# randyjhc/vit-colmap

Measured on AMD Instinct MI355X. Metric: images/sec extracted + pair-matches/sec (N×D brute-force NN), higher is better.
Workload: dtype bf16 (ViT) / u8+i32 (matcher); 1 GPU; configs[1]+configs[2]: DINOv2 ViT-S/14 extract of 50 640x480 images (512 keypoints, 384-D uint8 descriptors) then exhaustive mutual-NN + ratio matching of all pairs among the extracted images; images_total=50, images_rank0=50, num_keypoints=512, descriptor_dim=384, parallelism=images+pairs sharded x1

## Files before the change

vit_colmap_amd/csrc/gemm.hip:

```cpp
#include <hip/hip_runtime.h>
#include <stdint.h>

#include "../../include/vitcolmap_hip.h"
#include "common.h"
#include "device.h"

namespace {

typedef __bf16 v8bf __attribute__((ext_vector_type(8)));
typedef __bf16 v4bf __attribute__((ext_vector_type(4)));
typedef float v4f __attribute__((ext_vector_type(4)));

constexpr int BM = 128;
constexpr int BN = 128;
constexpr int BK = 64;
constexpr int kImg = 128 * 128;
constexpr int kStage = 2 * kImg;

enum { EPI_BIAS = 0, EPI_GELU = 1, EPI_RESIDUAL = 2, EPI_PATCH = 3, EPI_SWIGLU = 4 };
static_assert(EPI_BIAS == VC_EPI_BIAS && EPI_GELU == VC_EPI_GELU && EPI_RESIDUAL == VC_EPI_RESIDUAL && EPI_SWIGLU == VC_EPI_SWIGLU,
              "epilogue codes of the ABI");

__device__ __forceinline__ float gelu_erf(float x) {
  const float ax = __builtin_fabsf(x);
// ... 125 lines not shown
          *(v4bf*)(out + (size_t)m * H + n) = ov;
        }
      }
    }
    return;
  }
#pragma unroll
  for (int a = 0; a < 4; ++a) {
    const int n = n0 + wn * 64 + a * 16 + fq * 4;
    const v4bf bv = *(const v4bf*)(bias + n);
#pragma unroll
    for (int b = 0; b < 4; ++b) {
      const int m = m0 + wm * 64 + b * 16 + fr;
      if (m < M) {
        size_t o = (size_t)m * N + n;
        size_t ro = o;
        if (EPI == EPI_PATCH) {
          const int b_img = m / group;
          o = (size_t)(m + b_img + 1) * N + n;
          ro = (size_t)(m - b_img * group + 1) * N + n;
        }
        float v[4];
#pragma unroll
        for (int j = 0; j < 4; ++j) v[j] = acc[a][b][j] + (float)bv[j];
        if (EPI == EPI_GELU) {
#pragma unroll
          for (int j = 0; j < 4; ++j) v[j] = gelu_erf(v[j]);
        }
        if (EPI == EPI_RESIDUAL || EPI == EPI_PATCH) {
          const v4bf rv = *(const v4bf*)(res + ro);
#pragma unroll
          for (int j = 0; j < 4; ++j) v[j] += (float)rv[j];
        }
        v4bf ov;
#pragma unroll
        for (int j = 0; j < 4; ++j) ov[j] = (__bf16)v[j];
        *(v4bf*)(out + o) = ov;
      }
    }
  }
}


constexpr int G2M = 256, G2N = 256;
constexpr int kUnit2 = 128 * 128;
constexpr int kBuf2 = 4 * kUnit2;
constexpr int G256_LDS = 2 * kBuf2;
constexpr int kAhead2 = 6;

template <int EPI, bool CONV>
__global__ __launch_bounds__(512, 2) void gemm256_kernel(const __bf16* __restrict__ X, const __bf16* __restrict__ W,
                                                         const __bf16* __restrict__ bias, const __bf16* __restrict__ res,
                                                         __bf16* __restrict__ out, int M, int N, int K, int n_tiles_n,
                                                         int n_tiles, int cH, int cW, int cC, int ckw, int cdy0, int cdx0,
                                                         int cpar) {
  extern __shared__ __attribute__((aligned(1024))) uint8_t lds2[];
  const int tid = threadIdx.x, lane = tid & 63;
  const int wave = __builtin_amdgcn_readfirstlane(tid >> 6);
  const int wr = wave >> 2, wc = wave & 3;
  const int nk = K / BK;
  const int n_units = 4 * nk;
  for (int slot = blockIdx.x; slot < n_tiles; slot += gridDim.x) {
  int tile;
  {
    const int xcd = slot & 7, idx = slot >> 3;
    const int q = n_tiles >> 3, r = n_tiles & 7;
    tile = (xcd < r ? xcd * (q + 1) : r * (q + 1) + (xcd - r) * q) + idx;
  }
  const int tm = tile / n_tiles_n, tn = tile - tm * n_tiles_n;
  const int m0 = tm * G2M, n0 = tn * G2N;

  const uint32_t lds0 = vc::lds_addr(&lds2[0]);
  const int prow = lane >> 3, pchunk = (lane & 7) ^ prow;
  uint32_t voffx[2][2], voffw[2];
  uint32_t vtaps[2][2];
  const int n_taps = CONV ? K / cC : 1, tiles_per_tap = CONV ? cC / BK : 1;
#pragma unroll
  for (int i = 0; i < 2; ++i) {
    const int rho = (wave * 2 + i) * 8 + prow;
#pragma unroll
    for (int h = 0; h < 2; ++h) {
      const int xr = (rho < 64 ? rho : 128 + (rho - 64)) + 64 * h;
      if (CONV) {
        const int m = m0 + xr, hw = cH * cW;
        const int bimg = m / hw, rem = m - bimg * hw, py = rem / cW, px = rem - py * cW;
        uint32_t bits = 0;
        for (int t = 0; t < n_taps; ++t) {
          const int yy = py + cdy0 + t / ckw, xx = px + cdx0 + t % ckw;
          if (m < M && yy >= 0 && yy < cH && xx >= 0 && xx < cW) bits |= 1u << t;
        }
        vtaps[h][i] = bits;
        voffx[h][i] = (uint32_t)(((size_t)min(m, M - 1) * cC + pchunk * 8) * 2);
      } else {
        voffx[h][i] = (uint32_t)(((size_t)min(m0 + xr, M - 1) * K + pchunk * 8) * 2 - (size_t)min(m0, M - 1) * K * 2);
      }
    }
    const int wrow = EPI == EPI_SWIGLU ? rho : (rho >> 5) * 64 + (rho & 31);
    voffw[i] = (uint32_t)(((size_t)wrow * K + pchunk * 8) * 2);
  }
  const int H = N >> 1, j0 = tn * (G2N / 2);
  const char* const xbase = CONV ? (const char*)X : (const char*)(X + (size_t)min(m0, M - 1) * K);
  const char* const wbase = (const char*)(W + (size_t)(EPI == EPI_SWIGLU ? j0 : n0) * K);
  const size_t whalf = (size_t)(EPI == EPI_SWIGLU ? H : 32) * K * 2;
  auto issue = [&](int u) {
    if (u >= n_units) return;
    const int t = u >> 2, j = u & 3;
    const bool is_x = j == 0 || j == 3;
    const char* sb = is_x ? xbase + (size_t)t * (BK * 2) : wbase + (size_t)t * (BK * 2) + (j == 2 ? whalf : 0);
    int tap = 0;
    uint32_t zoff = 0, spos = 0;
    if (CONV && is_x) {
      tap = t / tiles_per_tap;
      const long long shift = ((long long)(cdy0 + tap / ckw) * cW + (cdx0 + tap % ckw)) * cC * 2;
      const long long sneg = shift < 0 ? shift : 0;
      spos = (uint32_t)(shift - sneg);
      sb = xbase + sneg + (long long)(t - tap * tiles_per_tap) * (BK * 2);
      zoff = (uint32_t)((long long)M * cC * 2 - sneg) + (uint32_t)pchunk * 16u;
    }
#pragma unroll
    for (int i = 0; i < 2; ++i) {
      uint32_t vo = j == 0 ? voffx[0][i] : (j == 3 ? voffx[1][i] : voffw[i]);
      if (CONV && is_x) vo = ((j == 0 ? vtaps[0][i] : vtaps[1][i]) >> tap) & 1u ? vo + spos : zoff;
      const uint32_t dst = lds0 + (uint32_t)(t & 1) * kBuf2 + (uint32_t)j * kUnit2 + (uint32_t)(wave * 2 + i) * 1024u;
      vc::lds_dma16(sb, vo, dst);
    }
  };

  v4f acc[4][8];
#pragma unroll
  for (int a = 0; a < 4; ++a)
#pragma unroll
    for (int b = 0; b < 8; ++b) acc[a][b] = (v4f){0.f, 0.f, 0.f, 0.f};

  const int fr = lane & 15, fq = lane >> 4;
  uint32_t xoff[2], woff[2];
#pragma unroll
  for (int ks = 0; ks < 2; ++ks) {
    const int ch = ks * 4 + fq;
    xoff[ks] = (uint32_t)(wr * 64 + fr) * 128u + (uint32_t)((ch ^ (fr & 7)) << 4);
    woff[ks] = (uint32_t)(wc * 32 + fr) * 128u + (uint32_t)((ch ^ (fr & 7)) << 4);
  }
  v8bf xf[2][4], wf[2][2][2];

  auto read_x = [&](const uint8_t* buf, int th) {
    const uint8_t* u = buf + (th == 0 ? 0 : 3) * kUnit2;
#pragma unroll
    for (int ks = 0; ks < 2; ++ks)
#pragma unroll
      for (int b = 0; b < 4; ++b) xf[ks][b] = *(const v8bf*)(u + xoff[ks] + b * 2048);
  };
  auto read_w = [&](const uint8_t* buf, int fh) {
    const uint8_t* u = buf + (1 + fh) * kUnit2;
#pragma unroll
    for (int ks = 0; ks < 2; ++ks)
#pragma unroll
      for (int a = 0; a < 2; ++a) wf[fh][ks][a] = *(const v8bf*)(u + woff[ks] + a * 2048);
  };
  auto barrier = []() { asm volatile("s_barrier" ::: "memory"); };
#define G2_MFMA(FH, TH)                                                                                      \
  asm volatile("s_waitcnt lgkmcnt(0)" ::: "memory");                                                         \
  __builtin_amdgcn_sched_barrier(0);                                                                         \
  __builtin_amdgcn_s_setprio(1);                                                                             \
  _Pragma("unroll") for (int ks = 0; ks < 2; ++ks)                                                           \
  _Pragma("unroll") for (int a = 0; a < 2; ++a)                                                              \
  _Pragma("unroll") for (int b = 0; b < 4; ++b)                                                              \
    acc[2 * (FH) + a][4 * (TH) + b] =                                                                        \
        __builtin_amdgcn_mfma_f32_16x16x32_bf16(wf[FH][ks][a], xf[ks][b], acc[2 * (FH) + a][4 * (TH) + b], 0, 0, 0); \
  __builtin_amdgcn_s_setprio(0);

#pragma unroll
  for (int u = 0; u < kAhead2; ++u) issue(u);
  if (nk > 1) asm volatile("s_waitcnt vmcnt(4)" ::: "memory"); else asm volatile("s_waitcnt vmcnt(0)" ::: "memory");
  barrier();
  if (wr == 1) barrier();

  for (int t = 0; t < nk; ++t) {
    const uint8_t* buf = lds2 + (size_t)(t & 1) * kBuf2;
    const int g = 4 * t;
    read_w(buf, 0);
    __builtin_amdgcn_sched_barrier(0);
    read_x(buf, 0);
    issue(g + kAhead2);
    barrier();
    G2_MFMA(0, 0)
    barrier();
    read_w(buf, 1);
    issue(g + 1 + kAhead2);
    barrier();
    G2_MFMA(1, 0)
    barrier();
    read_x(buf, 1);
    issue(g + 2 + kAhead2);
    barrier();
    G2_MFMA(1, 1)
    barrier();
    issue(g + 3 + kAhead2);
    if (t + 2 < nk) asm volatile("s_waitcnt vmcnt(4)" ::: "memory"); else asm volatile("s_waitcnt vmcnt(0)" ::: "memory");
    barrier();
    G2_MFMA(0, 1)
    barrier();
  }
  if (wr == 0) barrier();
#undef G2_MFMA

  typedef unsigned int v4u32 __attribute__((ext_vector_type(4)));
  typedef unsigned int v2u32 __attribute__((ext_vector_type(2)));
  typedef __bf16 v2bf16 __attribute__((ext_vector_type(2)));
  uint8_t* const ep = lds2 + (size_t)wave * 16384;
  const int lrow = lane >> 3, lslot = lane & 7;
  auto ep_at = [&](int row, int byte) { return ep + row * 128 + (byte ^ (((row >> 1) & 7) << 4)); };
  if (EPI == EPI_SWIGLU) {
    const size_t colh = (size_t)j0 + wc * 32;
#pragma unroll
    for (int a = 0; a < 2; ++a) {
      const v4bf bg = *(const v4bf*)(bias + colh + a * 16 + fq * 4), bv = *(const v4bf*)(bias + H + colh + a * 16 + fq * 4);
#pragma unroll
      for (int b = 0; b < 8; ++b) {
        const int row = 16 * b + fr;
        float v[4];
#pragma unroll
        for (int j = 0; j < 4; ++j) v[j] = swiglu_f32(acc[a][b][j] + (float)bg[j], acc[a + 2][b][j] + (float)bv[j]);
        const v2bf16 q0 = {(__bf16)v[0], (__bf16)v[1]}, q1 = {(__bf16)v[2], (__bf16)v[3]};
        *(v2u32*)ep_at(row >> 1, 64 * (row & 1) + 32 * a + 8 * fq) = (v2u32){*(const unsigned int*)&q0, *(const unsigned int*)&q1};
      }
    }
    asm volatile("s_waitcnt lgkmcnt(0)" ::: "memory");
#pragma unroll
    for (int i = 0; i < 8; ++i) {
      const int m = m0 + wr * 128 + 16 * i + (lane >> 2);
      const v4u32 o = *(const v4u32*)ep_at(8 * i + lrow, lslot * 16);
      if (m < M) *(v4u32*)(out + (size_t)m * H + colh + (lane & 3) * 8) = o;
    }
    asm volatile("s_barrier" ::: "memory");
    continue;
  }
  const size_t col0 = (size_t)n0 + wc * 64;
  if (EPI == EPI_RESIDUAL) {
    v4u32 rr[16];
#pragma unroll
    for (int i = 0; i < 16; ++i)
      rr[i] = *(const v4u32*)(res + (size_t)min(m0 + wr * 128 + 8 * i + lrow, M - 1) * N + col0 + lslot * 8);
#pragma unroll
    for (int i = 0; i < 16; ++i) *(v4u32*)ep_at(8 * i + lrow, lslot * 16) = rr[i];
    asm volatile("s_waitcnt lgkmcnt(0)" ::: "memory");
  }
#pragma unroll
  for (int a = 0; a < 4; ++a) {
    const v4bf bv = *(const v4bf*)(bias + col0 + a * 16 + fq * 4);
#pragma unroll
    for (int b = 0; b < 8; ++b) {
      uint8_t* const pp = ep_at(16 * b + fr, 32 * a + 8 * fq);
      float v[4];
#pragma unroll
      for (int j = 0; j < 4; ++j) v[j] = acc[a][b][j] + (float)bv[j];
      if (EPI == EPI_GELU) {
#pragma unroll
        for (int j = 0; j < 4; j += 2) {
          const v2f_t g = gelu_erf2((v2f_t){v[j], v[j + 1]});
          v[j] = g[0];
          v[j + 1] = g[1];
        }
      }
      if (EPI == EPI_RESIDUAL) {
        const v2u32 r8 = *(const v2u32*)pp;
#pragma unroll
        for (int j = 0; j < 2; ++j) {
          v[2 * j] += __uint_as_float(r8[j] << 16);
          v[2 * j + 1] += __uint_as_float(r8[j] & 0xffff0000u);
        }
      }
      const v2bf16 q0 = {(__bf16)v[0], (__bf16)v[1]}, q1 = {(__bf16)v[2], (__bf16)v[3]};
      *(v2u32*)pp = (v2u32){*(const unsigned int*)&q0, *(const unsigned int*)&q1};
    }
  }
  asm volatile("s_waitcnt lgkmcnt(0)" ::: "memory");
  if (CONV && cpar >= 0) {
    int mm = m0 + wr * 128 + lrow;
    int pb = mm / (cH * cW), py = (mm - pb * cH * cW) / cW, px = mm - pb * cH * cW - py * cW;
#pragma unroll
    for (int i = 0; i < 16; ++i) {
      const int row = 8 * i + lrow;
      const v4u32 o = *(const v4u32*)ep_at(row, lslot * 16);
      const size_t orow = ((size_t)pb * 2 * cH + 2 * py + (cpar >> 1)) * (2 * cW) + 2 * px + (cpar & 1);
      if (mm < M) *(v4u32*)(out + orow * N + col0 + lslot * 8) = o;
      mm += 8;
      px += 8;
      while (px >= cW) { px -= cW; if (++py == cH) { py = 0; ++pb; } }
    }
  } else {
#pragma unroll
    for (int i = 0; i < 16; ++i) {
      const int row = 8 * i + lrow, m = m0 + wr * 128 + row;
      const v4u32 o = *(const v4u32*)ep_at(row, lslot * 16);
      if (m < M) *(v4u32*)(out + (size_t)m * N + col0 + lslot * 8) = o;
    }
  }
  asm volatile("s_barrier" ::: "memory");
  }
}

constexpr int XK = 384;
constexpr int XKS = XK / 16;
constexpr int XStage = XKS * 1024;
constexpr int XNS = 3;
constexpr int XPF = XNS - 1;
constexpr int XMaxN = 4096;
constexpr int XRows = 256;
constexpr int XChunk = 32 * 128;
constexpr int XOffBias = XNS * XStage;
constexpr int XOffStage = XOffBias + XMaxN * 4;
constexpr int XLds = XOffStage + 8 * 2 * XChunk;

typedef float v16f __attribute__((ext_vector_type(16)));
typedef uint32_t v4u __attribute__((ext_vector_type(4)));

constexpr uint32_t kGtLo = (127 - 14) << 7;
constexpr uint32_t kGtN = 17 * 128;
constexpr int kGtBytes = (int)kGtN * 2 * 2;

__device__ __forceinline__ uint32_t f32_to_bf16_rne(float v) {
  uint32_t u = __float_as_uint(v);
  u += 0x7fffu + ((u >> 16) & 1u);
  return u >> 16;
}
__global__ void gelu_table_kernel(uint16_t* __restrict__ tab) {
  const uint32_t i = blockIdx.x * blockDim.x + threadIdx.x;
  if (i >= kGtN * 2) return;
  const uint32_t k = i >> 1, sign = i & 1;
  const float x = __uint_as_float(((sign << 15) | (kGtLo + k)) << 16);
  const float y = 0.5f * x * (1.0f + erff(x * 0.70710678118654752f));
  tab[i] = (uint16_t)f32_to_bf16_rne(y);
}

constexpr int XReadAhead = 8;
constexpr int XIssue0 = 1;
constexpr int XIssueStep = 8;
template <int EPI, bool LN, bool GT>
__global__ __launch_bounds__(512, 1) void xs_kernel(const __bf16* __restrict__ X, const uint8_t* __restrict__ Wp,
                                                    const float* __restrict__ biasf, const __bf16* res,
                                                    __bf16* out, int M, int N, int n_nb, int n_stages, float eps,
                                                    const uint16_t* __restrict__ gelu_tab) {
  __shared__ __attribute__((aligned(1024))) uint8_t lds[XLds];
  const int tid = threadIdx.x, lane = tid & 63;
  const int wave = __builtin_amdgcn_readfirstlane(tid >> 6);
  const int r = lane & 31, h = lane >> 5;

  const int G = gridDim.x, bid = blockIdx.x;
  const int s0 = (int)((long long)n_stages * bid / G), s1 = (int)((long long)n_stages * (bid + 1) / G);
  const int n = s1 - s0;
  if (n <= 0) return;

  float* bias_l = (float*)(lds + XOffBias);
  for (int i = tid; i < N; i += 512) bias_l[i] = biasf[i];
  uint8_t* const gt_l = lds + XOffBias + ((N * 4 + 15) & ~15);
  if (GT)
    for (int i = tid; i < kGtBytes / 4; i += 512) ((uint32_t*)gt_l)[i] = ((const uint32_t*)gelu_tab)[i];

  const uint32_t lds0 = vc::lds_addr(&lds[0]);
  int inb = s0 % n_nb, islot = 0, ileft = n;
  const uint32_t lane_off16 = (uint32_t)lane * 16u;
  auto issue_piece = [&](int i) {
    const uint8_t* sbase = Wp + (size_t)inb * XStage + (size_t)(wave * 3 + i) * 1024;
    const uint32_t dst = lds0 + (uint32_t)islot * XStage + (uint32_t)(wave * 3 + i) * 1024u;
    vc::lds_dma16(sbase, lane_off16, dst);
    if (i == 2) {
      if (ileft > 1) { --ileft; inb = inb + 1 == n_nb ? 0 : inb + 1; }
      islot = islot + 1 == XNS ? 0 : islot + 1;
    }
  };
  auto issue = [&]() {
#pragma unroll
    for (int i = 0; i < 3; ++i) issue_piece(i);
  };
#pragma unroll
  for (int j = 0; j < XPF; ++j) issue();

  v8bf xf[XKS];
  typedef float v2f __attribute__((ext_vector_type(2)));
  const int prow = lane >> 3;
  auto x_issue = [&](int mt) {
#pragma unroll
    for (int p = 0; p < 4; ++p) {
      const int m = min(mt * XRows + wave * 32 + 8 * p + prow, M - 1);
      const uint8_t* src = (const uint8_t*)X + (size_t)m * (XK * 2) + (lane & 7) * 16;
#pragma unroll
      for (int c = 0; c < XK / 64; ++c) *(v4u*)&xf[4 * c + p] = *(const v4u*)(src + c * 128);
    }
  };
  auto x_finish = [&]() {
    uint8_t* const tp = lds + XOffStage + wave * (2 * XChunk);
    const int fsw = (r >> 1) & 7;
#pragma unroll
    for (int c = 0; c < XK / 64; ++c) {
#pragma unroll
      for (int p = 0; p < 4; ++p) {
        const int row = 8 * p + prow;
        *(v4u*)(tp + row * 128 + (((lane & 7) ^ ((row >> 1) & 7)) << 4)) = *(const v4u*)&xf[4 * c + p];
      }
#pragma unroll
      for (int k4 = 0; k4 < 4; ++k4)
        xf[4 * c + k4] = *(const v8bf*)(tp + r * 128 + (((2 * k4 + h) ^ fsw) << 4));
    }
    if (LN) {
      auto expand = [](uint32_t u) { return (v2f){__uint_as_float(u << 16), __uint_as_float(u & 0xffff0000u)}; };
      v2f s2 = {0.f, 0.f};
#pragma unroll
      for (int ks = 0; ks < XKS; ++ks) {
        const v4u u = *(const v4u*)&xf[ks];
#pragma unroll
        for (int j = 0; j < 4; ++j) s2 += expand(u[j]);
      }
      float sum = s2[0] + s2[1];
      sum += __shfl_xor(sum, 32);
      const float mean = sum * (1.0f / XK);
      const v2f mean2 = {mean, mean};
#pragma unroll
      for (int ks = 0; ks < XKS; ++ks) asm volatile("" : "+v"(xf[ks]));
      v2f q2 = {0.f, 0.f};
#pragma unroll
      for (int ks = 0; ks < XKS; ++ks) {
        const v4u u = *(const v4u*)&xf[ks];
#pragma unroll
        for (int j = 0; j < 4; ++j) { const v2f d = expand(u[j]) - mean2; q2 = __builtin_elementwise_fma(d, d, q2); }
      }
      float q = q2[0] + q2[1];
      q += __shfl_xor(q, 32);
      const float rstd = __builtin_amdgcn_rsqf(q * (1.0f / XK) + eps);
      const v2f rstd2 = {rstd, rstd};
#pragma unroll
      for (int ks = 0; ks < XKS; ++ks) asm volatile("" : "+v"(xf[ks]));
#pragma unroll
      for (int ks = 0; ks < XKS; ++ks) {
        const v4u u = *(const v4u*)&xf[ks];
#pragma unroll
        for (int j = 0; j < 4; ++j) {
          const v2f y = (expand(u[j]) - mean2) * rstd2;
          xf[ks][2 * j] = (__bf16)y[0];
          xf[ks][2 * j + 1] = (__bf16)y[1];
        }
      }
    }
  };

  const __amdgpu_buffer_rsrc_t out_rs = __builtin_amdgcn_make_buffer_rsrc(out, 0, (int)((size_t)M * N * 2), 0x00020000);
  uint8_t* const tr_out = lds + XOffStage + wave * (2 * XChunk);
  uint8_t* const tr_res = tr_out + 2048;
  const int crow = lane >> 2, cch = lane & 3;
  const int rsw = (r >> 2) & 3;
  v4u resq[2];
  auto load_res = [&](int m_base, int nb) {
    if (EPI == EPI_RESIDUAL) {
#pragma unroll
      for (int q = 0; q < 2; ++q)
        resq[q] = *(const v4u*)(res + (size_t)min(m_base + crow + 16 * q, M - 1) * N + nb * 32 + cch * 8);
    }
  };
  v16f pa;
  float ev[16];
  uint32_t ep[8];
  v4u eo[2];
  int pm_base = 0, pnb = 0;
  auto res_to_lds = [&]() {
    if (EPI == EPI_RESIDUAL) {
#pragma unroll
      for (int q = 0; q < 2; ++q) {
        const int row = crow + 16 * q;
        *(v4u*)(tr_res + row * 64 + ((cch ^ ((row >> 2) & 3)) << 4)) = resq[q];
      }
    }
  };
  uint32_t gq[8];
  uint32_t gres[8];
  uint32_t gbad = 0;
  auto slice = [&](int sl) {
    if (EPI == EPI_GELU && GT) {
      typedef __bf16 v2bf __attribute__((ext_vector_type(2)));
      if (sl < 4) {
        const int g = sl;
        const v2bf lo = {(__bf16)pa[4 * g], (__bf16)pa[4 * g + 1]}, hi = {(__bf16)pa[4 * g + 2], (__bf16)pa[4 * g + 3]};
        ep[2 * g] = *(const uint32_t*)&lo;
        ep[2 * g + 1] = *(const uint32_t*)&hi;
        if (sl == 0) gbad = 0;
      }
      if (sl >= 4 && sl < 12) {
        const int qd = sl - 4;
        const uint32_t b0 = ep[qd] & 0xffffu, b1 = ep[qd] >> 16;
        const uint32_t k0 = (b0 & 0x7fffu) - kGtLo, k1 = (b1 & 0x7fffu) - kGtLo;
        gbad = max(gbad, max(k0, k1));
        const uint32_t a0 = min(k0, kGtN - 1) * 4 + ((b0 >> 15) << 1), a1 = min(k1, kGtN - 1) * 4 + ((b1 >> 15) << 1);
        gq[2 * (qd & 3)] = *(const uint16_t*)(gt_l + a0);
        gq[2 * (qd & 3) + 1] = *(const uint16_t*)(gt_l + a1);
      }
      if (sl >= 7 && sl < 15) {
        const int qd = sl - 7;
        gres[qd] = gq[2 * (qd & 3)] | (gq[2 * (qd & 3) + 1] << 16);
      }
      if (sl == 15) {
        if (__any(gbad >= kGtN)) {
#pragma unroll
          for (int qd = 0; qd < 8; ++qd) {
            const v2f_t xin = {__uint_as_float(ep[qd] << 16), __uint_as_float(ep[qd] & 0xffff0000u)};
            const v2f_t y = gelu_erf2(xin);
            const v2bf o = {(__bf16)y[0], (__bf16)y[1]};
            ep[qd] = *(const uint32_t*)&o;
          }
        } else {
#pragma unroll
          for (int qd = 0; qd < 8; ++qd) ep[qd] = gres[qd];
        }
      }
      if (sl == 16) {
#pragma unroll
        for (int i = 0; i < 4; ++i) {
          const auto sw = __builtin_amdgcn_permlane32_swap(ep[i], ep[i + 4], false, false);
          ep[i] = sw[0];
          ep[i + 4] = sw[1];
        }
      }
      if (sl == 17) {
        *(v4u*)(tr_out + r * 64 + (((2 * h) ^ rsw) << 4)) = (v4u){ep[0], ep[1], ep[4], ep[5]};
        *(v4u*)(tr_out + r * 64 + (((2 * h + 1) ^ rsw) << 4)) = (v4u){ep[2], ep[3], ep[6], ep[7]};
      }
      if (sl == 19) {
#pragma unroll
        for (int q = 0; q < 2; ++q) {
          const int row = crow + 16 * q;
          eo[q] = *(const v4u*)(tr_out + row * 64 + ((cch ^ ((row >> 2) & 3)) << 4));
        }
      }
      if (sl == 22) {
#pragma unroll
        for (int q = 0; q < 2; ++q) {
          const int row = crow + 16 * q;
          __builtin_amdgcn_raw_buffer_store_b128(eo[q], out_rs, (int)(((size_t)(pm_base + row) * N + pnb * 32 + cch * 8) * 2), 0, 0);
        }
      }
      return;
    }
    if (sl < 8) {
      const int j0 = 2 * sl;
      if (EPI == EPI_GELU) {
        const v2f_t y = gelu_erf2((v2f_t){pa[j0], pa[j0 + 1]});
        ev[j0] = y[0];
        ev[j0 + 1] = y[1];
      } else if (EPI == EPI_RESIDUAL) {
        if ((sl & 1) == 0) {
          const int g = sl >> 1;
          const v4bf rv = *(const v4bf*)(tr_res + r * 64 + ((g ^ rsw) << 4) + 8 * h);
#pragma unroll
          for (int j = 0; j < 4; ++j) ev[4 * g + j] = pa[4 * g + j] + (float)rv[j];
        }
      } else {
        ev[j0] = pa[j0];
        ev[j0 + 1] = pa[j0 + 1];
      }
    } else if (sl < 12) {
      const int g = sl - 8;
      typedef __bf16 v2bf __attribute__((ext_vector_type(2)));
      const v2bf lo = {(__bf16)ev[4 * g], (__bf16)ev[4 * g + 1]}, hi = {(__bf16)ev[4 * g + 2], (__bf16)ev[4 * g + 3]};
      ep[2 * g] = *(const uint32_t*)&lo;
      ep[2 * g + 1] = *(const uint32_t*)&hi;
    } else if (sl == 12) {
#pragma unroll
      for (int i = 0; i < 4; ++i) {
        const auto sw = __builtin_amdgcn_permlane32_swap(ep[i], ep[i + 4], false, false);
        ep[i] = sw[0];
        ep[i + 4] = sw[1];
      }
    } else if (sl == 13) {
      *(v4u*)(tr_out + r * 64 + (((2 * h) ^ rsw) << 4)) = (v4u){ep[0], ep[1], ep[4], ep[5]};
      *(v4u*)(tr_out + r * 64 + (((2 * h + 1) ^ rsw) << 4)) = (v4u){ep[2], ep[3], ep[6], ep[7]};
    } else if (sl == 15) {
#pragma unroll
      for (int q = 0; q < 2; ++q) {
        const int row = crow + 16 * q;
        eo[q] = *(const v4u*)(tr_out + row * 64 + ((cch ^ ((row >> 2) & 3)) << 4));
      }
    } else if (sl == 19) {
#pragma unroll
      for (int q = 0; q < 2; ++q) {
        const int row = crow + 16 * q;
        __builtin_amdgcn_raw_buffer_store_b128(eo[q], out_rs, (int)(((size_t)(pm_base + row) * N + pnb * 32 + cch * 8) * 2), 0, 0);
      }
    }
  };

  v16f acc;
  int mt_cur = -1, slot = 0;
  int mt = s0 / n_nb, nb = s0 - mt * n_nb;
  for (int i = 0; i < n; ++i) {
    if (i >= 2) {
      if (EPI == EPI_RESIDUAL) asm volatile("s_waitcnt vmcnt(7)" ::: "memory");
      else asm volatile("s_waitcnt vmcnt(5)" ::: "memory");
    } else {
      asm volatile("s_waitcnt vmcnt(3)" ::: "memory");
    }
    asm volatile("s_waitcnt lgkmcnt(0)\n\ts_barrier" ::: "memory");
    const bool pending = i > 0;
    if (pending) res_to_lds();
    const bool reload = mt != mt_cur;
    const int m_base = mt * XRows + wave * 32;
    if (reload) {
      x_issue(mt);
      if (pending) {
#pragma unroll
        for (int sl = 0; sl < XKS; ++sl) slice(sl);
      }
      x_finish();
      mt_cur = mt;
    }
    load_res(m_base, nb);
    const uint8_t* st = lds + slot * XStage + lane * 16;
    {
      const float* bl = bias_l + nb * 32 + 4 * h;
#pragma unroll
      for (int g = 0; g < 4; ++g) {
        const v4f bv = *(const v4f*)(bl + 8 * g);
#pragma unroll
        for (int j = 0; j < 4; ++j) acc[4 * g + j] = bv[j];
      }
    }
    {
      constexpr int XRD = (EPI == EPI_GELU && GT) ? 6 : XReadAhead;
      v8bf wf[XKS];
#pragma unroll
      for (int ks = 0; ks < XRD; ++ks) wf[ks] = *(const v8bf*)(st + ks * 1024);
      __builtin_amdgcn_sched_barrier(0);
      if (pending && !reload) {
#pragma unroll
        for (int ks = 0; ks < XKS; ++ks) {
          acc = __builtin_amdgcn_mfma_f32_32x32x16_bf16(wf[ks], xf[ks], acc, 0, 0, 0);
          if (ks + XRD < XKS) wf[ks + XRD] = *(const v8bf*)(st + (ks + XRD) * 1024);
          slice(ks);
          if (ks == XIssue0 || ks == XIssue0 + XIssueStep || ks == XIssue0 + 2 * XIssueStep)
            issue_piece((ks - XIssue0) / XIssueStep);
          __builtin_amdgcn_sched_barrier(0);
        }
      } else {
#pragma unroll
        for (int ks = 0; ks < XKS; ++ks) {
          acc = __builtin_amdgcn_mfma_f32_32x32x16_bf16(wf[ks], xf[ks], acc, 0, 0, 0);
          if (ks + XRD < XKS) wf[ks + XRD] = *(const v8bf*)(st + (ks + XRD) * 1024);
          if (ks == XIssue0 || ks == XIssue0 + XIssueStep || ks == XIssue0 + 2 * XIssueStep)
            issue_piece((ks - XIssue0) / XIssueStep);
          __builtin_amdgcn_sched_barrier(0);
        }
      }
    }
    pa = acc;
    pm_base = m_base;
    pnb = nb;
    slot = slot + 1 == XNS ? 0 : slot + 1;
    if (++nb == n_nb) { nb = 0; ++mt; }
  }
  res_to_lds();
#pragma unroll
  for (int sl = 0; sl < XKS; ++sl) slice(sl);
  asm volatile("s_waitcnt vmcnt(0)" ::: "memory");
}

__global__ __launch_bounds__(256) void xs_prepare_kernel(const float* __restrict__ W, const float* __restrict__ b,
                                                         const float* __restrict__ gamma, const float* __restrict__ beta,
                                                         int N, __bf16* __restrict__ Wp, float* __restrict__ biasf) {
  const int lane = threadIdx.x & 63;
  const int nfeat = blockIdx.x * 4 + (threadIdx.x >> 6);
  if (nfeat >= N) return;
  const int nb = nfeat >> 5, rr = nfeat & 31;
  float dot = 0.f;
  for (int k = lane; k < XK; k += 64) {
    const float w = W[(size_t)nfeat * XK + k];
    const float wg = gamma ? w * gamma[k] : w;
    if (beta) dot += w * beta[k];
    const int ks = k >> 4, hh = (k >> 3) & 1, j = k & 7;
    Wp[(((size_t)nb * XKS + ks) * 64 + hh * 32 + rr) * 8 + j] = (__bf16)wg;
  }
#pragma unroll
  for (int o = 32; o > 0; o >>= 1) dot += __shfl_xor(dot, o);
  if (lane == 0) biasf[nfeat] = (b ? b[nfeat] : 0.f) + dot;
}


constexpr int MStage = 2 * XStage;
constexpr int MNS = 2;

constexpr int M2OffB1 = MNS * MStage;
constexpr int M2OffGt = M2OffB1 + 1536 * 4;
constexpr int M2OffB2 = M2OffGt + 8704;
constexpr int M2OffTrA = M2OffB2 + 1536;
constexpr int M2OffTrB = M2OffTrA + 4 * XChunk;
constexpr int M2OffG = M2OffTrB + 4 * XChunk;
constexpr int M2Lds = M2OffG + 2 * 4 * 2048;
static_assert(M2Lds <= 160 * 1024, "fused MLP: LDS budget");

constexpr int M2ReadAhead = 6;
constexpr int M2PiecesA = 3;
constexpr int M2Issue0 = 1;
constexpr int M2IssueStep = 3;
constexpr int M2IssueStepB = 2;
__global__ __launch_bounds__(512, 2) void mlp2_kernel(__bf16* __restrict__ X, const uint8_t* __restrict__ Wm,
                                                      const float* __restrict__ b1f, const float* __restrict__ b2f,
                                                      int M, int n_chunks, int n_tiles, float eps,
                                                      const uint16_t* __restrict__ gelu_tab) {
  __shared__ __attribute__((aligned(1024))) uint8_t lds[M2Lds];
  const int tid = threadIdx.x, lane = tid & 63;
  const int wave = __builtin_amdgcn_readfirstlane(tid >> 6);
  const bool roleB = wave >= 4;
  const int pairw = wave & 3;
  const int r = lane & 31, h = lane >> 5;
  const int G = gridDim.x, bid = blockIdx.x;
  const int my_tiles = bid < n_tiles ? (n_tiles - bid + G - 1) / G : 0;
  const int n = my_tiles * n_chunks;
  if (n <= 0) return;

  float* const b1_l = (float*)(lds + M2OffB1);
  float* const b2_l = (float*)(lds + M2OffB2);
  uint8_t* const gt_l = lds + M2OffGt;
  for (int i = tid; i < n_chunks * 32; i += 512) b1_l[i] = b1f[i];
  for (int i = tid; i < XK; i += 512) b2_l[i] = b2f[i];
  for (int i = tid; i < kGtBytes / 4; i += 512) ((uint32_t*)gt_l)[i] = ((const uint32_t*)gelu_tab)[i];

  const uint32_t lds0 = vc::lds_addr(&lds[0]);
  const uint32_t lane_off = (uint32_t)lane * 16u;
  constexpr int NA = M2PiecesA, NB = 12 - NA;
  auto issue_piece = [&](int c1, int c2, int slot, int i) {
    const int role = wave >> 2, q = wave & 3;
    if (i >= (role ? NB : NA)) return;
    const int id = role ? 4 * NA + q * NB + i : q * NA + i;
    const int half = id >= 24, idx = id - 24 * half;
    const int c = half ? c2 : c1;
    const uint8_t* sbase = Wm + (size_t)c * MStage + (size_t)half * XStage + (size_t)idx * 1024;
    const uint32_t dst = lds0 + (uint32_t)slot * MStage + (uint32_t)half * XStage + (uint32_t)idx * 1024u;
    vc::lds_dma16(sbase, lane_off, dst);
  };
  auto issue = [&](int c1, int c2, int slot) {
#pragma unroll
    for (int i = 0; i < (NA > NB ? NA : NB); ++i) issue_piece(c1, c2, slot, i);
  };
  typedef __bf16 v2bf __attribute__((ext_vector_type(2)));
  typedef float v2f __attribute__((ext_vector_type(2)));

  int chunk = 0, slot = 0, tile = bid;
  auto chunk_of = [&](int j) { return j % n_chunks; };
  auto issue_stage = [&](int j, int slot_) {
    const int c1 = chunk_of(min(max(j, 0), n - 1)), c2 = chunk_of(min(max(j - 2, 0), n - 1));
    issue(c1, c2, slot_);
  };
  issue_stage(0, 0);
  if (!roleB) {
    v8bf xf[XKS];
    uint8_t* const tp = lds + M2OffTrA + pairw * XChunk;
    const int prow = lane >> 3;
    v16f hprev;
    uint32_t pb[8], gq[8], gres[8], gbad = 0;
    auto gelu_slice = [&](int sl, int parity) {
      if (sl < 4) {
        const int g = sl;
        const v2bf lo = {(__bf16)hprev[4 * g], (__bf16)hprev[4 * g + 1]}, hi = {(__bf16)hprev[4 * g + 2], (__bf16)hprev[4 * g + 3]};
        pb[2 * g] = *(const uint32_t*)&lo;
        pb[2 * g + 1] = *(const uint32_t*)&hi;
        if (sl == 0) gbad = 0;
      }
      if (sl >= 4 && sl < 12) {
        const int qd = sl - 4;
        const uint32_t b0 = pb[qd] & 0xffffu, b1 = pb[qd] >> 16;
        const uint32_t k0 = (b0 & 0x7fffu) - kGtLo, k1 = (b1 & 0x7fffu) - kGtLo;
        gbad = max(gbad, max(k0, k1));
        gq[2 * (qd & 3)] = *(const uint16_t*)(gt_l + min(k0, kGtN - 1) * 4 + ((b0 >> 15) << 1));
        gq[2 * (qd & 3) + 1] = *(const uint16_t*)(gt_l + min(k1, kGtN - 1) * 4 + ((b1 >> 15) << 1));
      }
      if (sl >= 7 && sl < 15) {
        const int qd = sl - 7;
        gres[qd] = gq[2 * (qd & 3)] | (gq[2 * (qd & 3) + 1] << 16);
      }
      if (sl == 15) {
        if (__any(gbad >= kGtN)) {
#pragma unroll
          for (int qd = 0; qd < 8; ++qd) {
            const v2f_t y = gelu_erf2((v2f_t){__uint_as_float(pb[qd] << 16), __uint_as_float(pb[qd] & 0xffff0000u)});
            const v2bf o = {(__bf16)y[0], (__bf16)y[1]};
            gres[qd] = *(const uint32_t*)&o;
          }
        }
      }
      if (sl == 16) {
        uint8_t* const gb = lds + M2OffG + (parity * 4 + pairw) * 2048 + lane * 16;
        *(v4u*)gb = (v4u){gres[0], gres[1], gres[2], gres[3]};
        *(v4u*)(gb + 1024) = (v4u){gres[4], gres[5], gres[6], gres[7]};
      }
    };
    for (int i = 0; i <= n + 1; ++i) {
      asm volatile("s_waitcnt vmcnt(0)" ::: "memory");
      asm volatile("s_waitcnt lgkmcnt(0)\n\ts_barrier" ::: "memory");
      const bool do_issue = i <= n;
      const int nc1 = chunk_of(min(max(i + 1, 0), n - 1)), nc2 = chunk_of(min(max(i - 1, 0), n - 1));
      if (do_issue && !(i < n && i > 0)) issue_stage(i + 1, slot ^ 1);
      if (i < n) {
        if (chunk == 0) {
          const int m0w = tile * 128 + pairw * 32;
#pragma unroll
          for (int p = 0; p < 4; ++p) {
            const int m = min(m0w + 8 * p + prow, M - 1);
            const uint8_t* src = (const uint8_t*)X + (size_t)m * (XK * 2) + (lane & 7) * 16;
#pragma unroll
            for (int c = 0; c < XK / 64; ++c) *(v4u*)&xf[4 * c + p] = *(const v4u*)(src + c * 128);
          }
          const int fsw = (r >> 1) & 7;
#pragma unroll
          for (int c = 0; c < XK / 64; ++c) {
#pragma unroll
            for (int p = 0; p < 4; ++p) {
              const int row = 8 * p + prow;
              *(v4u*)(tp + row * 128 + (((lane & 7) ^ ((row >> 1) & 7)) << 4)) = *(const v4u*)&xf[4 * c + p];
            }
#pragma unroll
            for (int k4 = 0; k4 < 4; ++k4)
              xf[4 * c + k4] = *(const v8bf*)(tp + r * 128 + (((2 * k4 + h) ^ fsw) << 4));
          }
          auto expand = [](uint32_t u) { return (v2f){__uint_as_float(u << 16), __uint_as_float(u & 0xffff0000u)}; };
          v2f s2 = {0.f, 0.f};
#pragma unroll
          for (int ks = 0; ks < XKS; ++ks) {
            const v4u u = *(const v4u*)&xf[ks];
#pragma unroll
            for (int j = 0; j < 4; ++j) s2 += expand(u[j]);
          }
          float sum = s2[0] + s2[1];
          sum += __shfl_xor(sum, 32);
          const float mean = sum * (1.0f / XK);
          const v2f mean2 = {mean, mean};
#pragma unroll
          for (int ks = 0; ks < XKS; ++ks) asm volatile("" : "+v"(xf[ks]));
          v2f q2 = {0.f, 0.f};
#pragma unroll
          for (int ks = 0; ks < XKS; ++ks) {
            const v4u u = *(const v4u*)&xf[ks];
#pragma unroll
            for (int j = 0; j < 4; ++j) { const v2f d = expand(u[j]) - mean2; q2 = __builtin_elementwise_fma(d, d, q2); }
          }
          float q = q2[0] + q2[1];
          q += __shfl_xor(q, 32);
          const float rstd = __builtin_amdgcn_rsqf(q * (1.0f / XK) + eps);
          const v2f rstd2 = {rstd, rstd};
#pragma unroll
          for (int ks = 0; ks < XKS; ++ks) asm volatile("" : "+v"(xf[ks]));
#pragma unroll
          for (int ks = 0; ks < XKS; ++ks) {
            const v4u u = *(const v4u*)&xf[ks];
#pragma unroll
            for (int j = 0; j < 4; ++j) {
              const v2f y = (expand(u[j]) - mean2) * rstd2;
              xf[ks][2 * j] = (__bf16)y[0];
              xf[ks][2 * j + 1] = (__bf16)y[1];
            }
          }
        }
        const uint8_t* st = lds + slot * MStage + lane * 16;
        v16f hacc;
        {
          const float* bl = b1_l + chunk * 32 + 4 * h;
#pragma unroll
          for (int g = 0; g < 4; ++g) {
            const v4f bv = *(const v4f*)(bl + 8 * g);
#pragma unroll
            for (int j = 0; j < 4; ++j) hacc[4 * g + j] = bv[j];
          }
        }
        {
          constexpr int RD = M2ReadAhead;
          v8bf wf[XKS];
#pragma unroll
          for (int ks = 0; ks < RD; ++ks) wf[ks] = *(const v8bf*)(st + ks * 1024);
          __builtin_amdgcn_sched_barrier(0);
          __builtin_amdgcn_s_setprio(1);
          if (i > 0) {
#pragma unroll
            for (int ks = 0; ks < XKS; ++ks) {
              hacc = __builtin_amdgcn_mfma_f32_32x32x16_bf16(wf[ks], xf[ks], hacc, 0, 0, 0);
              if (ks + RD < XKS) wf[ks + RD] = *(const v8bf*)(st + (ks + RD) * 1024);
              gelu_slice(ks, (i - 1) & 1);
              if (ks >= M2Issue0 && ks < M2Issue0 + NA * M2IssueStep && (ks - M2Issue0) % M2IssueStep == 0 && do_issue)
                issue_piece(nc1, nc2, slot ^ 1, (ks - M2Issue0) / M2IssueStep);
              __builtin_amdgcn_sched_barrier(0);
            }
          } else {
#pragma unroll
            for (int ks = 0; ks < XKS; ++ks) {
              hacc = __builtin_amdgcn_mfma_f32_32x32x16_bf16(wf[ks], xf[ks], hacc, 0, 0, 0);
              if (ks + RD < XKS) wf[ks + RD] = *(const v8bf*)(st + (ks + RD) * 1024);
              __builtin_amdgcn_sched_barrier(0);
            }
          }
        }
        __builtin_amdgcn_s_setprio(0);
        hprev = hacc;
        if (++chunk == n_chunks) { chunk = 0; tile += G; }
      } else if (i == n) {
#pragma unroll
        for (int sl = 0; sl < XKS; ++sl) gelu_slice(sl, (i - 1) & 1);
      }
      slot ^= 1;
    }
  } else {
    v16f oacc[12];
    const __amdgpu_buffer_rsrc_t out_rs = __builtin_amdgcn_make_buffer_rsrc(X, 0, (int)((size_t)M * XK * 2), 0x00020000);
    const int crow = lane >> 2, cch = lane & 3;
    const int rsw = (r >> 2) & 3;
    uint8_t* const tr_out = lds + M2OffTrB + pairw * XChunk;
    uint8_t* const tr_res = tr_out + 2048;
    int pchunk = 0;
    for (int i = 0; i <= n + 1; ++i) {
      asm volatile("s_waitcnt vmcnt(0)" ::: "memory");
      asm volatile("s_waitcnt lgkmcnt(0)\n\ts_barrier" ::: "memory");
      const bool do_issue = i <= n;
      const int nc1 = chunk_of(min(max(i + 1, 0), n - 1)), nc2 = chunk_of(min(max(i - 1, 0), n - 1));
      if (i >= 2) {
        if (pchunk == 0) {
#pragma unroll
          for (int ob = 0; ob < 12; ++ob)
#pragma unroll
            for (int j = 0; j < 16; ++j) oacc[ob][j] = 0.f;
        }
        const uint8_t* gb = lds + M2OffG + ((i & 1) * 4 + pairw) * 2048 + lane * 16;
        const v8bf g_s0 = *(const v8bf*)gb, g_s1 = *(const v8bf*)(gb + 1024);
        const uint8_t* st2 = lds + slot * MStage + XStage + lane * 16;
        {
          constexpr int RD = M2ReadAhead;
          v8bf wf[24];
#pragma unroll
          for (int q = 0; q < RD; ++q) wf[q] = *(const v8bf*)(st2 + q * 1024);
#pragma unroll
          for (int q = 0; q < 24; ++q) {
            oacc[q >> 1] = __builtin_amdgcn_mfma_f32_32x32x16_bf16(wf[q], (q & 1) ? g_s1 : g_s0, oacc[q >> 1], 0, 0, 0);
            if (q + RD < 24) wf[q + RD] = *(const v8bf*)(st2 + (q + RD) * 1024);
            constexpr int BSTEP = NB <= 6 ? M2IssueStep : M2IssueStepB;
            if (q >= M2Issue0 && q < M2Issue0 + NB * BSTEP && (q - M2Issue0) % BSTEP == 0 && do_issue)
              issue_piece(nc1, nc2, slot ^ 1, (q - M2Issue0) / BSTEP);
          }
        }
        if (pchunk == n_chunks - 1) {
          const int m0w = tile * 128 + pairw * 32;
#pragma unroll 1
          for (int ob = 0; ob < 12; ++ob) {
            v4u resq[2];
#pragma unroll
            for (int q = 0; q < 2; ++q)
              resq[q] = *(const v4u*)(X + (size_t)min(m0w + crow + 16 * q, M - 1) * XK + ob * 32 + cch * 8);
#pragma unroll
            for (int q = 0; q < 2; ++q) {
              const int row = crow + 16 * q;
              *(v4u*)(tr_res + row * 64 + ((cch ^ ((row >> 2) & 3)) << 4)) = resq[q];
            }
            v16f oa;
            switch (ob) {
#define VC_OB(k) case k: oa = oacc[k]; break;
              VC_OB(0) VC_OB(1) VC_OB(2) VC_OB(3) VC_OB(4) VC_OB(5) VC_OB(6) VC_OB(7) VC_OB(8) VC_OB(9) VC_OB(10)
              default: oa = oacc[11]; break;
#undef VC_OB
            }
// ... 276 lines not shown
```

Baseline: 7570 images/s.

## Stream residual via LDS DMA and stagger wave barriers in xs GEMM

Residual tiles are now loaded directly into a double-buffered per-wave LDS region with LDS DMA, replacing the register load followed by an LDS store. The weight ring grows from three to four stages while keeping a prefetch distance of two. The per-iteration barrier is split so that waves 0-3 sync at the top of the loop and waves 4-7 sync mid-way through the K loop, using a new inline-asm helper with conditional waitcnt. The aim is to cut register pressure and barrier stalls and to overlap the residual fetch with the MFMA loop, at the cost of more LDS and fragile hand-written vmcnt accounting.

```diff
diff --git a/vit_colmap_amd/csrc/gemm.hip b/vit_colmap_amd/csrc/gemm.hip
--- a/vit_colmap_amd/csrc/gemm.hip
+++ b/vit_colmap_amd/csrc/gemm.hip
@@ -451,14 +451,16 @@
 constexpr int XK = 384;
 constexpr int XKS = XK / 16;
 constexpr int XStage = XKS * 1024;
-constexpr int XNS = 3;
-constexpr int XPF = XNS - 1;
+constexpr int XNS = 4;
+constexpr int XPF = 2;
 constexpr int XMaxN = 4096;
 constexpr int XRows = 256;
 constexpr int XChunk = 32 * 128;
 constexpr int XOffBias = XNS * XStage;
 constexpr int XOffStage = XOffBias + XMaxN * 4;
-constexpr int XLds = XOffStage + 8 * 2 * XChunk;
+constexpr int XResBuf = 32 * 64;
+constexpr int XWaveStage = XChunk + XResBuf;
+constexpr int XLds = XOffStage + 8 * XWaveStage;
 
 typedef float v16f __attribute__((ext_vector_type(16)));
 typedef uint32_t v4u __attribute__((ext_vector_type(4)));
@@ -483,7 +485,28 @@
 
 constexpr int XReadAhead = 8;
 constexpr int XIssue0 = 1;
+constexpr int XResWait = 18;
 constexpr int XIssueStep = 8;
+template <int N1, int N2, bool LGKM>
+__device__ __forceinline__ void xs_wait_barrier(int mode) {
+  asm volatile(
+      "s_cmp_eq_u32 %0, 0\n\t"
+      "s_cbranch_scc1 .Lxs_pass_%=\n\t"
+      "s_cmp_eq_u32 %0, 2\n\t"
+      "s_cbranch_scc1 .Lxs_two_%=\n\t"
+      "s_waitcnt vmcnt(%1)\n\t"
+      "s_branch .Lxs_bar_%=\n"
+      ".Lxs_two_%=:\n\t"
+      "s_waitcnt vmcnt(%2)\n"
+      ".Lxs_bar_%=:\n\t"
+      "s_waitcnt lgkmcnt(%3)\n\t"
+      "s_barrier\n"
+      ".Lxs_pass_%=:"
+      :
+      : "s"(__builtin_amdgcn_readfirstlane(mode)), "n"(N1), "n"(N2), "n"(LGKM ? 0 : 15)
+      : "memory", "scc");
+}
+
 template <int EPI, bool LN, bool GT>
 __global__ __launch_bounds__(512, 1) void xs_kernel(const __bf16* __restrict__ X, const uint8_t* __restrict__ Wp,
                                                     const float* __restrict__ biasf, const __bf16* res,
@@ -537,7 +560,7 @@
     }
   };
   auto x_finish = [&]() {
-    uint8_t* const tp = lds + XOffStage + wave * (2 * XChunk);
+    uint8_t* const tp = lds + XOffStage + wave * XWaveStage;
     const int fsw = (r >> 1) & 7;
 #pragma unroll
     for (int c = 0; c < XK / 64; ++c) {
@@ -592,16 +615,18 @@
   };
 
   const __amdgpu_buffer_rsrc_t out_rs = __builtin_amdgcn_make_buffer_rsrc(out, 0, (int)((size_t)M * N * 2), 0x00020000);
-  uint8_t* const tr_out = lds + XOffStage + wave * (2 * XChunk);
-  uint8_t* const tr_res = tr_out + 2048;
+  uint8_t* const tr_out = lds + XOffStage + wave * XWaveStage;
+  const uint8_t* tr_res = tr_out + 2048;
   const int crow = lane >> 2, cch = lane & 3;
   const int rsw = (r >> 2) & 3;
-  v4u resq[2];
-  auto load_res = [&](int m_base, int nb) {
+  const uint32_t tr_res_a = lds0 + (uint32_t)XOffStage + (uint32_t)wave * XWaveStage + 2048u;
+  const int rch = cch ^ ((crow >> 2) & 3);
+  uint32_t rbuf = 0;
+  auto issue_res = [&](int m_base, int nb) {
     if (EPI == EPI_RESIDUAL) {
 #pragma unroll
       for (int q = 0; q < 2; ++q)
-        resq[q] = *(const v4u*)(res + (size_t)min(m_base + crow + 16 * q, M - 1) * N + nb * 32 + cch * 8);
+        vc::lds_dma16(res + (size_t)min(m_base + crow + 16 * q, M - 1) * N + nb * 32 + rch * 8, tr_res_a + rbuf + q * 1024u);
     }
   };
   v16f pa;
@@ -609,15 +634,6 @@
   uint32_t ep[8];
   v4u eo[2];
   int pm_base = 0, pnb = 0;
-  auto res_to_lds = [&]() {
-    if (EPI == EPI_RESIDUAL) {
-#pragma unroll
-      for (int q = 0; q < 2; ++q) {
-        const int row = crow + 16 * q;
-        *(v4u*)(tr_res + row * 64 + ((cch ^ ((row >> 2) & 3)) << 4)) = resq[q];
-      }
-    }
-  };
   uint32_t gq[8];
   uint32_t gres[8];
   uint32_t gbad = 0;
@@ -737,16 +753,12 @@
   v16f acc;
   int mt_cur = -1, slot = 0;
   int mt = s0 / n_nb, nb = s0 - mt * n_nb;
+  const bool late = wave >= 4;
+  asm volatile("s_waitcnt vmcnt(3)\n\ts_waitcnt lgkmcnt(0)\n\ts_barrier" ::: "memory");
+  constexpr int XResOps = EPI == EPI_RESIDUAL ? 2 : 0;
   for (int i = 0; i < n; ++i) {
-    if (i >= 2) {
-      if (EPI == EPI_RESIDUAL) asm volatile("s_waitcnt vmcnt(7)" ::: "memory");
-      else asm volatile("s_waitcnt vmcnt(5)" ::: "memory");
-    } else {
-      asm volatile("s_waitcnt vmcnt(3)" ::: "memory");
-    }
-    asm volatile("s_waitcnt lgkmcnt(0)\n\ts_barrier" ::: "memory");
+    xs_wait_barrier<3, 5 + XResOps, true>(late || i == 0 ? 0 : i >= 2 ? 2 : 1);
     const bool pending = i > 0;
-    if (pending) res_to_lds();
     const bool reload = mt != mt_cur;
     const int m_base = mt * XRows + wave * 32;
     if (reload) {
@@ -758,7 +770,7 @@
       x_finish();
       mt_cur = mt;
     }
-    load_res(m_base, nb);
+    issue_res(m_base, nb);
     const uint8_t* st = lds + slot * XStage + lane * 16;
     {
       const float* bl = bias_l + nb * 32 + 4 * h;
@@ -778,31 +790,35 @@
       if (pending && !reload) {
 #pragma unroll
         for (int ks = 0; ks < XKS; ++ks) {
+          if (ks == XKS / 2) xs_wait_barrier<2 + XResOps, 2 + XResOps, false>(late && i + 1 < n ? 1 : 0);
           acc = __builtin_amdgcn_mfma_f32_32x32x16_bf16(wf[ks], xf[ks], acc, 0, 0, 0);
           if (ks + XRD < XKS) wf[ks + XRD] = *(const v8bf*)(st + (ks + XRD) * 1024);
           slice(ks);
           if (ks == XIssue0 || ks == XIssue0 + XIssueStep || ks == XIssue0 + 2 * XIssueStep)
             issue_piece((ks - XIssue0) / XIssueStep);
+          if (EPI == EPI_RESIDUAL && ks == XResWait) asm volatile("s_waitcnt vmcnt(3)" ::: "memory");
           __builtin_amdgcn_sched_barrier(0);
         }
       } else {
 #pragma unroll
         for (int ks = 0; ks < XKS; ++ks) {
+          if (ks == XKS / 2) xs_wait_barrier<2 + XResOps, 2 + XResOps, false>(late && i + 1 < n ? 1 : 0);
           acc = __builtin_amdgcn_mfma_f32_32x32x16_bf16(wf[ks], xf[ks], acc, 0, 0, 0);
           if (ks + XRD < XKS) wf[ks + XRD] = *(const v8bf*)(st + (ks + XRD) * 1024);
           if (ks == XIssue0 || ks == XIssue0 + XIssueStep || ks == XIssue0 + 2 * XIssueStep)
             issue_piece((ks - XIssue0) / XIssueStep);
+          if (EPI == EPI_RESIDUAL && ks == XResWait) asm volatile("s_waitcnt vmcnt(3)" ::: "memory");
           __builtin_amdgcn_sched_barrier(0);
         }
       }
     }
     pa = acc;
+    if (EPI == EPI_RESIDUAL) { tr_res = tr_out + 2048 + rbuf; rbuf ^= (uint32_t)XResBuf; }
     pm_base = m_base;
     pnb = nb;
     slot = slot + 1 == XNS ? 0 : slot + 1;
     if (++nb == n_nb) { nb = 0; ++mt; }
   }
-  res_to_lds();
 #pragma unroll
   for (int sl = 0; sl < XKS; ++sl) slice(sl);
   asm volatile("s_waitcnt vmcnt(0)" ::: "memory");
```

Result: no change. 7576 images/s, median of 2 (+0.1%).
